# AI4Science-WestlakeU/wdno

Measured on AMD Instinct MI355X. Metric: diffusion train steps/sec, 2D smoke U-Net (8 samples per GPU per step), higher is better.
Workload: dtype f32

## Files before the change

### include/wdno_hip.h

```cpp
#ifndef WDNO_HIP_H
#define WDNO_HIP_H
#include <stdint.h>
#include <stddef.h>

#ifdef __cplusplus
extern "C" {
#endif

typedef void* wdno_stream_t;

enum { WDNO_OK = 0, WDNO_EINVAL = -1, WDNO_ELAUNCH = -2, WDNO_EUNSUPPORTED = -3, WDNO_EWORKSPACE = -4 };

#define WDNO_AMAX_SLOTS 64
#define WDNO_AMAX_STRIDE 16
#define WDNO_AMAX_FLOATS (WDNO_AMAX_SLOTS * WDNO_AMAX_STRIDE)
const char* wdno_strerror(int code);
int wdno_version(void);
const char* wdno_last_hip_error(void);
int wdno_set_debug(int mode);

typedef struct {
  int nd;
  int mode;
  int L;
// ... 81 lines not shown
int wdno_conv_wgrad_f16x3_param(const void* xh, const void* xl, const float* sx, const void* dyh, const void* dyl, const float* sdy,
                                const void* pixel_table, float* dw, int Kn, int Cn, void* ws, size_t ws_bytes,
                                const wdno_conv_geom* g, wdno_stream_t s);
#define WDNO_WGRAD_REDUCE_MAX 40
typedef struct wdno_wgrad_reduce_item {
  const float* ws; float* dw;
  int n, splits;
  int K8, C8, kw, ntap, Kn, Cn;
  int tiled;
  int reserved;
} wdno_wgrad_reduce_item;
int wdno_conv_wgrad_partials(const void* xh, const void* xl, const float* sx, const void* dyh, const void* dyl, const float* sdy,
                             const void* pixel_table, float* dw, int Kn, int Cn, void* ws, size_t ws_bytes,
                             const wdno_conv_geom* g, wdno_wgrad_reduce_item* item, wdno_stream_t s);
int wdno_wgrad_reduce_multi(const wdno_wgrad_reduce_item* items, int n_items, wdno_stream_t s);
size_t wdno_conv_wgrad_ws_bytes(const wdno_conv_geom* g);
int wdno_conv_wgrad(const float* x, const float* dy, float* dwp, void* ws, size_t ws_bytes,
                    const wdno_conv_geom* g, wdno_stream_t s);
#define WDNO_ROWS_SUM_MAX 64
typedef struct wdno_rows_sum_item {
  const void* part; float* out;
  int rows, stride, col0, ncols;
  int is_double, reserved;
} wdno_rows_sum_item;
int wdno_rows_sum_multi(const wdno_rows_sum_item* items, int n_items, wdno_stream_t s);
size_t wdno_colsum_ws_bytes(int64_t P, int C);
int wdno_colsum(const float* in, float* out, int64_t P, int C, void* ws, size_t ws_bytes, wdno_stream_t s);

int wdno_cast_bf16(const float* x, void* out16, int64_t rows, int C, int C8, wdno_stream_t s);
int wdno_cast_bf16_colsum(const float* x, void* out16, float* colsum_out, void* ws, size_t ws_bytes, int64_t rows, int C, int C8, wdno_stream_t s);
// ... 307 lines not shown
```

### wdno_amd/_lib.py

```python
import contextlib
import ctypes as C
import os

import torch

HERE = os.path.dirname(os.path.abspath(__file__))
LIB_PATH = os.path.join(HERE, 'libwdno_hip.so')

P = C.c_void_p
I = C.c_int
L = C.c_int64
F = C.c_float
Z = C.c_size_t


class DwtDesc(C.Structure):
    _fields_ = [('nd', I), ('mode', I), ('L', I), ('n_img', I), ('in_dims', I * 3), ('out_dims', I * 3),
                ('cs_img', L), ('cs_band', L), ('cs0', L), ('cs1', L)]


class ConvGeom(C.Structure):
    _fields_ = [(k, I) for k in ('N', 'D', 'H', 'W', 'C', 'OD', 'OH', 'OW', 'K', 'kd', 'kh', 'kw', 'sd', 'sh', 'sw',
                                 'pd', 'ph', 'pw', 'YD', 'YH', 'YW', 'osd', 'osh', 'osw', 'ood', 'ooh', 'oow')]

# ... 23 lines not shown
ATTN_FAMILIES = ('mfma24', 'mfma', 'mfma64', 'tiled', 'tiled_staged', 'tiled_unstaged', 'big', 'rows')


class LinAttnPlan(C.Structure):
    _fields_ = [(k, I) for k in ('kstats_chunks', 'ctx_chunks', 'token_tiles', 'family', 'rc')]


class LayerNormPlan(C.Structure):
    _fields_ = [(k, I) for k in ('tpr', 'vpl', 'rows_per_block', 'blocks', 'max_rows_walk', 'rc')]


class ConvWgradPlan(C.Structure):
    _fields_ = [(k, I) for k in ('family', 'bm', 'bn', 'splits', 'pix_per_split', 'splitpair', 'reduce_tiled', 'items', 'grid')]


CONV_FAMILIES = ('fp32', 'h3', 'h3d', 'h3t', 'h3t_stem')
WGRAD_FAMILIES = ('h3', 'h3d', 'h3w', 'h3s')


class RowsSumItem(C.Structure):
    _fields_ = [('part', C.c_void_p), ('out', C.c_void_p), ('rows', I), ('stride', I), ('col0', I), ('ncols', I), ('is_double', I), ('reserved', I)]


class BurgersDesc(C.Structure):
    _fields_ = [(k, I) for k in ('N', 's', 'nx0', 'nt_f', 'nxf', 'steps', 'record_time', 'f_time', 'num_t', 'sub_s', 'out_cols', 'waves',
                                 'points')] + [(k, F) for k in ('c', 'd', 'dm', 'dt')]


class BurgersGenerateDesc(C.Structure):
    _fields_ = [(k, I) for k in ('N', 's', 't', 'steps', 'record_time', 'f_time', 'num_t', 'st', 'sx', 'f_rows', 'cols', 'waves', 'points',
# ... 75 lines not shown
    'wdno_amax_multi': (I, [P, I, I, P]),
    'wdno_pack_split_weight_multi': (I, [P, I, I, P]),
    'wdno_conv_fwd_f16x3': (I, [P, P, P, P, P, P, P, P, P, PG, P]),
    'wdno_conv_fwd_f16x3_amax': (I, [P, P, P, P, P, P, P, P, P, P, PG, P]),
    'wdno_conv_fwd_f16x3_ws': (I, [P, P, P, P, P, P, P, P, P, P, PG, P, Z, P]),
    'wdno_conv_fwd_split_ws_bytes': (Z, [PG]),
    'wdno_conv_wgrad_f16x3_ws_bytes': (Z, [PG]),
    'wdno_conv_fwd_plan': (I, [PG, I, I, Z, P]),
    'wdno_conv_wgrad_plan': (I, [PG, I, I, I, P]),
    'wdno_conv_pixel_table': (I, [P, PG, P]),
    'wdno_conv_wgrad_f16x3': (I, [P, P, P, P, P, P, P, P, P, Z, PG, P]),
    'wdno_conv_wgrad_f16x3_param': (I, [P, P, P, P, P, P, P, P, I, I, P, Z, PG, P]),
    'wdno_conv_wgrad_partials': (I, [P, P, P, P, P, P, P, P, I, I, P, Z, PG, P, P]),
    'wdno_wgrad_reduce_multi': (I, [P, I, P]),
    'wdno_rows_sum_multi': (I, [P, I, P]),
    'wdno_cast_bf16': (I, [P, P, L, I, I, P]),
    'wdno_cast_bf16_colsum': (I, [P, P, P, P, Z, L, I, I, P]),
    'wdno_conv_fwd_bf16': (I, [P, P, P, P, P, P, PG, P]),
    'wdno_conv_fwd_f16x3_zbox': (I, [P, P, P, P, P, P, P, P, P, P, PG, P, P]),
    'wdno_conv_fwd_bf16_ex': (I, [P, P, P, P, P, I, P, PG, P, P]),
    'wdno_conv_wgrad_bf16_param': (I, [P, P, P, P, I, I, P, Z, PG, P]),
    'wdno_conv_wgrad_ws_bytes': (Z, [PG]),
    'wdno_conv_wgrad': (I, [P, P, P, P, Z, PG, P]),
    'wdno_colsum_ws_bytes': (Z, [L, I]),
    'wdno_colsum': (I, [P, P, L, I, P, Z, P]),
    'wdno_groupnorm_ws_bytes': (Z, [L, L, I, I]),
    'wdno_groupnorm_stats_floats': (Z, [L, I, I]),
    'wdno_groupnorm_act_fwd': (I, [P, P, P, P, P, P, L, L, I, I, F, I, P, Z, P]),
    'wdno_groupnorm_act_fwd_amax': (I, [P, P, P, P, P, P, P, L, L, I, I, F, I, P, Z, P]),
    'wdno_groupnorm_act_bwd': (I, [P, P, P, P, P, P, P, P, P, L, L, I, I, I, P, Z, P]),
# ... 131 lines not shown
```

### wdno_amd/csrc/conv_common.h

```cpp
#pragma once
#include "common.h"

typedef float f32x16 __attribute__((ext_vector_type(16)));

#define BK 32
#define LDS_STRIDE 36

struct ConvP {
  wdno_conv_geom g;
  int R;
  int nchunk;
  int nsteps;
  int64_t P;
  int identity_out;
  int debug;
  int tiles_n;
  int ntiles;
  int ksplit;
  float* amax_rec;
  int tsplit;
  float* split_ws;
  size_t split_ws_bytes;
  int zb_blocks, zb_d, zb_h;
  int out_bf16;
// ... 17 lines not shown
static inline int check_geom(const wdno_conv_geom* g) {
  if (!g) return WDNO_EINVAL;
  if (g->N <= 0 || g->D <= 0 || g->H <= 0 || g->W <= 0 || g->C <= 0 || g->K <= 0) return WDNO_EINVAL;
  if (g->OD <= 0 || g->OH <= 0 || g->OW <= 0 || g->kd <= 0 || g->kh <= 0 || g->kw <= 0) return WDNO_EINVAL;
  if (g->sd <= 0 || g->sh <= 0 || g->sw <= 0 || g->osd <= 0 || g->osh <= 0 || g->osw <= 0) return WDNO_EINVAL;
  if ((g->C & 3) || (g->K & 3)) return WDNO_EUNSUPPORTED;
  if ((g->OD - 1) * g->osd + g->ood >= g->YD || (g->OH - 1) * g->osh + g->ooh >= g->YH || (g->OW - 1) * g->osw + g->oow >= g->YW)
    return WDNO_EINVAL;
  return WDNO_OK;
}
#include "debug_modes.h"
void wdno_wgrad_h3d_plan(const wdno_conv_geom* g, int* bm, int* bn, int* splits, int* pix_per_split, int* splitpair = nullptr);
int wdno_conv_wgrad_h3_dma(const void* xh, const void* xl, const void* dyh, const void* dyl, const float* sx, const float* sdy,
                           const void* table, float* wsf, const wdno_conv_geom* g, hipStream_t st);
int wdno_wgrad_h3d_describe(const wdno_conv_geom* g, wdno_wgrad_plan* out);
struct ConvFwdChoice {
  wdno_conv_plan plan;
  int kw;
  int sp;
};
static inline int conv_persistent_grid(int64_t items) {
  int grid = wdno_num_cus() & ~7;
  if (grid < 8) grid = 8;
  if (items < grid) grid = (int)items;
  return grid;
}
int wdno_conv_fwd_fp32_plan(const wdno_conv_geom* g, wdno_conv_plan* out);
int wdno_conv_fwd_h3_dma_choose(const ConvP& p, bool lp, ConvFwdChoice& c);
int wdno_conv_fwd_h3_dma(const void* xh, const void* xl, const void* wh, const void* wl, const float* sx, const float* sw,
                         const float* bias, const float* residual, float* y, ConvP& p, const ConvFwdChoice& c, hipStream_t st);
// ... 36 lines not shown
```

### wdno_amd/csrc/conv_h3.hip

```cpp
#include "conv_common.h"
#include <type_traits>
#include <algorithm>

typedef _Float16 half8 __attribute__((ext_vector_type(8)));
typedef __bf16 bf16x8 __attribute__((ext_vector_type(8)));
template <bool LP>
__device__ __forceinline__ f32x16 mfma_16(half8 a, half8 b, f32x16 c) {
  if constexpr (LP) return __builtin_amdgcn_mfma_f32_32x32x16_bf16(__builtin_bit_cast(bf16x8, a), __builtin_bit_cast(bf16x8, b), c, 0, 0, 0);
  else return __builtin_amdgcn_mfma_f32_32x32x16_f16(a, b, c, 0, 0, 0);
}

#define HBK 32
#define HST 40

template <bool RECORD>
__global__ __launch_bounds__(256) void amax_kernel(const float* __restrict__ x, int64_t n, unsigned* __restrict__ out) {
  __shared__ float red[4];
  const int64_t n4 = n >> 2;
  const float4* x4 = reinterpret_cast<const float4*>(x);
  float m = 0.f;
  const int64_t stride = (int64_t)gridDim.x * 1024;
  for (int64_t k0 = (int64_t)blockIdx.x * 1024 + threadIdx.x; k0 < n4; k0 += stride) {
    float4 v[4];
#pragma unroll
// ... 1107 lines not shown
  return wdno_check_launch();
}

extern "C" int wdno_conv_wgrad_partials(const void* xh, const void* xl, const float* sx, const void* dyh, const void* dyl, const float* sdy,
                                        const void* pixel_table, float* dw, int Kn, int Cn, void* ws, size_t ws_bytes,
                                        const wdno_conv_geom* g, wdno_wgrad_reduce_item* item, wdno_stream_t s) {
  WDNO_REQUIRE(g && item && dw && Kn > 0 && Cn > 0 && Kn <= g->K && Cn <= g->C);
  int splits = 0;
  int rc = wgrad_h3_partials(xh, xl, sx, dyh, dyl, sdy, pixel_table, nullptr, ws, ws_bytes, g, as_stream(s), &splits);
  if (rc) return rc;
  const int64_t n = (int64_t)g->kd * g->kh * g->K * (int64_t)g->kw * g->C;
  if (n >= 0x7fffffff) return WDNO_EUNSUPPORTED;
  item->ws = (const float*)ws; item->dw = dw; item->n = (int)n; item->splits = splits; item->K8 = g->K; item->C8 = g->C; item->kw = g->kw;
  item->ntap = g->kd * g->kh; item->Kn = Kn; item->Cn = Cn; item->tiled = wgrad_h3_reduce_tiled(splits, g, Kn, Cn) ? 1 : 0;
  return wdno_check_launch();
}

extern "C" int wdno_conv_wgrad_bf16_param(const void* x16, const void* dy16, const void* pixel_table, float* dw, int Kn, int Cn, void* ws,
                                          size_t ws_bytes, const wdno_conv_geom* g, wdno_stream_t s) {
  WDNO_REQUIRE(g && Kn > 0 && Cn > 0 && Kn <= g->K && Cn <= g->C);
  hipStream_t st = as_stream(s);
  int splits = 0;
  int rc = wgrad_h3_partials(x16, nullptr, nullptr, dy16, nullptr, nullptr, pixel_table, nullptr, ws, ws_bytes, g, st, &splits);
  if (rc) return rc;
  const int64_t n = (int64_t)g->kd * g->kh * g->K * (int64_t)g->kw * g->C;
  wgrad_h3_reduce_launch((const float*)ws, dw, n, splits, g, Kn, Cn, st);
  return wdno_check_launch();
}

#define PS_LDS_FLOATS 10240
// ... 170 lines not shown
```

### wdno_amd/csrc/conv_wgrad_h3d.hip

```cpp
#include "conv_common.h"
#include <type_traits>

typedef _Float16 half8 __attribute__((ext_vector_type(8)));
typedef __bf16 bf16x8 __attribute__((ext_vector_type(8)));
typedef int int4v __attribute__((ext_vector_type(4)));
#define WD_OOB 0x7ffffff0
template <bool LP>
__device__ __forceinline__ f32x16 mfma_16(half8 a, half8 b, f32x16 c) {
  if constexpr (LP) return __builtin_amdgcn_mfma_f32_32x32x16_bf16(__builtin_bit_cast(bf16x8, a), __builtin_bit_cast(bf16x8, b), c, 0, 0, 0);
  else return __builtin_amdgcn_mfma_f32_32x32x16_f16(a, b, c, 0, 0, 0);
}

struct WgradDP {
  ConvP c;
  int tiles_k, tiles_r, splits, nsteps;
  int items;
  int pix_per_split;
  int xcd_chunk;
  int splitpair, n_a;
};

__device__ __forceinline__ int4v wd_rsrc(const void* ptr, unsigned bytes) {
  uint64_t a = reinterpret_cast<uint64_t>(ptr);
  int4v r;
// ... 12 lines not shown
  return v;
}
template <int NCH>
__device__ __forceinline__ half8 wd_frag(const char* plane, int lane_off, int pix0, int ch0) {
  typedef short short4v __attribute__((ext_vector_type(4)));
  typedef short4v __attribute__((address_space(3))) * lds_s4;
  const char* p0 = plane + lane_off + (pix0 / 4) * (NCH * 64) + (ch0 / 32) * 256;
  short4v a = __builtin_amdgcn_ds_read_tr16_b64_v4i16((lds_s4)(p0));
  short4v b = __builtin_amdgcn_ds_read_tr16_b64_v4i16((lds_s4)(p0 + NCH * 64));
  typedef short short8v __attribute__((ext_vector_type(8)));
  short8v c = __builtin_shufflevector(a, b, 0, 1, 2, 3, 4, 5, 6, 7);
  return __builtin_bit_cast(half8, c);
}

template <int BM, int BN, int NS, bool LP>
__global__ __launch_bounds__(512) void conv_wgrad_h3d_kernel(const _Float16* __restrict__ xh, const _Float16* __restrict__ xl,
                                                              const _Float16* __restrict__ dyh, const _Float16* __restrict__ dyl,
                                                              const float* __restrict__ sx, const float* __restrict__ sdy,
                                                              const int4v* __restrict__ table, float* __restrict__ ws, WgradDP wp,
                                                              unsigned x_bytes, unsigned dy_bytes, unsigned tbl_bytes) {
  constexpr int TM = BM / 64, TN = BN / 64;
  constexpr int ACH = BM / 8, BCH = BN / 8;
  constexpr int A_PLANE = 32 * ACH * 16, B_PLANE = 32 * BCH * 16;
  constexpr int NPL = LP ? 1 : 2;
  constexpr int A_LO = A_PLANE, B_HI = NPL * A_PLANE, B_LO = B_HI + B_PLANE;
  constexpr int STAGE = NPL * (A_PLANE + B_PLANE);
  constexpr int APC = A_PLANE / 1024, BPC = B_PLANE / 1024;
  constexpr int NPAIR = APC + BPC;
  static_assert(NPAIR % 4 == 0, "pieces are dealt to four producer waves");
  constexpr int R = NPAIR / 4;
  constexpr int PW = NPL * R;
  constexpr int LA = 2;
  static_assert(R + (NS - 2) * (R + PW) <= 63, "vmcnt is a 6-bit counter");
  extern __shared__ __attribute__((aligned(1024))) char smem[];
  const ConvP& p = wp.c;
  const wdno_conv_geom& g = p.g;
  const int tid = threadIdx.x;
  const int wave = __builtin_amdgcn_readfirstlane(tid >> 6), lane = tid & 63;
  int it_first, it_stride, my_items;
  if (wp.xcd_chunk > 0) {
    const int xcd = (int)blockIdx.x & 7, idx = (int)blockIdx.x >> 3;
    const int beg = xcd * wp.xcd_chunk, end = min(beg + wp.xcd_chunk, wp.items);
    it_stride = (int)gridDim.x >> 3;
    it_first = beg + idx;
    my_items = it_first < end ? (end - it_first + it_stride - 1) / it_stride : 0;
  } else {
    it_first = (int)blockIdx.x; it_stride = (int)gridDim.x;
    my_items = (wp.items - it_first + it_stride - 1) / it_stride;
  }
  const int ntap = g.kd * g.kh;
  auto decode_item = [&](int t, int& tile_k, int& tap, int& tile_r, int& split) {
    int id = it_first + t * it_stride;
    tile_r = id % wp.tiles_r; id /= wp.tiles_r;
    tap = id % ntap; id /= ntap;
    tile_k = id % wp.tiles_k;
    split = id / wp.tiles_k;
  };

  if (wave >= 4) {
    const int pq = wave - 4;
    int4v rxh = wd_rsrc(xh, x_bytes), rxl = wd_rsrc(xl, x_bytes), rdh = wd_rsrc(dyh, dy_bytes), rdl = wd_rsrc(dyl, dy_bytes);
    int4v rtb = wd_rsrc(table, tbl_bytes);
// ... 222 lines not shown
      float* orow = out + (int64_t)kk * p.R;
#pragma unroll
      for (int b = 0; b < TN; ++b) {
#pragma unroll
        for (int e4 = 0; e4 < 4; ++e4) {
          const int rr = tile_r * BN + n_base + b * 32 + 8 * e4 + 4 * hh;
          if (rr < p.R)
            *reinterpret_cast<float4*>(orow + rr) = make_float4(acc[a][b][4 * e4] * inv, acc[a][b][4 * e4 + 1] * inv, acc[a][b][4 * e4 + 2] * inv, acc[a][b][4 * e4 + 3] * inv);
        }
      }
    }
  }
}

template <int NS, bool LP>
__global__ __launch_bounds__(512) void conv_wgrad_h3w_kernel(const _Float16* __restrict__ xh, const _Float16* __restrict__ xl,
                                                              const _Float16* __restrict__ dyh, const _Float16* __restrict__ dyl,
                                                              const float* __restrict__ sx, const float* __restrict__ sdy,
                                                              const int4v* __restrict__ table, float* __restrict__ ws, WgradDP wp,
                                                              unsigned x_bytes, unsigned dy_bytes, unsigned tbl_bytes) {
  constexpr int KW = 3, BM = 64, CT = 64;
  constexpr int TM = 2, TN = 3;
  constexpr int ACH = BM / 8, XCH = CT / 8;
  constexpr int XROWS = 32 + KW - 1;
  constexpr int A_PLANE = 32 * ACH * 16, W_PLANE = 5 * 1024, B_PLANE = 2 * W_PLANE;
  constexpr int ZROWS = 9 * (XCH * 64);
  constexpr int NDY = 2;
  constexpr int NPL = LP ? 1 : 2;
  constexpr int A_LO = NDY * A_PLANE, B_HI = NPL * NDY * A_PLANE, B_LO = B_HI + B_PLANE;
  constexpr int STAGE = NPL * (NDY * A_PLANE + B_PLANE);
  constexpr int APC = A_PLANE / 1024, WPC = W_PLANE / 1024;
  static_assert(APC == 4 && WPC == 5, "ordinary items: pairs 0-3 dy, 4-8 window 0, 9-13 window 1; split-pair items: 0-3 dy 0, 4-7 dy 1, 8-12 window 0, 13-17 window 1");
  constexpr int LA = 2;
  extern __shared__ __attribute__((aligned(1024))) char smem[];
  const ConvP& p = wp.c;
  const wdno_conv_geom& g = p.g;
  const int tid = threadIdx.x;
  const int wave = __builtin_amdgcn_readfirstlane(tid >> 6), lane = tid & 63;
  int it_first, it_stride, my_items;
  if (wp.xcd_chunk > 0) {
    const int xcd = (int)blockIdx.x & 7, idx = (int)blockIdx.x >> 3;
    const int beg = xcd * wp.xcd_chunk, end = min(beg + wp.xcd_chunk, wp.items);
    it_stride = (int)gridDim.x >> 3;
    it_first = beg + idx;
    my_items = it_first < end ? (end - it_first + it_stride - 1) / it_stride : 0;
  } else {
    it_first = (int)blockIdx.x; it_stride = (int)gridDim.x;
    my_items = (wp.items - it_first + it_stride - 1) / it_stride;
  }
  const int ntap = g.kd * g.kh, npair = wp.splitpair ? ntap >> 1 : (ntap + 1) >> 1;
  auto decode_item = [&](int t, int& tile_k, int& tile_c, int (&tp)[2], int (&sp)[2]) {
    int id = it_first + t * it_stride;
    if (id < wp.n_a) {
      tile_c = id % wp.tiles_r; id /= wp.tiles_r;
      const int q = id % npair; id /= npair;
      tile_k = id % wp.tiles_k;
      sp[0] = sp[1] = id / wp.tiles_k;
      tp[0] = 2 * q; tp[1] = 2 * q + 1;
    } else {
      id -= wp.n_a;
      tile_c = id % wp.tiles_r; id /= wp.tiles_r;
      tile_k = id % wp.tiles_k;
// ... 57 lines not shown
            i_off[j] = k * 2;
          } else {
            i_ok[j] = row[j] < XROWS;
            i_off[j] = g.pw * g.C + tc * CT + chk[j];
          }
        }
      };
      if (my_items > 0) { load_item_r(); load_item_p(); }
      int4v rec[LA + 1][R];
      bool rok[LA + 1][R];
      auto fetch = [&](auto SLOT) {
        constexpr int S = decltype(SLOT)::value;
        const bool live = rc.t < my_items;
#pragma unroll
        for (int j = 0; j < R; ++j) {
          const int pm = r_pbeg[slot[j]] + rc.s * 32 + row[j] - (pq + 4 * j < APCT ? 0 : g.pw);
          rok[S][j] = live && pm >= 0 && pm < (int)p.P;
          rec[S][j] = wd_load_rec(rtb, rok[S][j] ? pm * 16 : WD_OOB);
        }
        if (live && ++rc.s == wp.nsteps) { rc.s = 0; if (++rc.t < my_items) load_item_r(); }
      };
      auto issue = [&](auto SLOT, int stage) {
        constexpr int S = decltype(SLOT)::value;
        const bool live = pc.t < my_items;
        const unsigned sb = lds0 + stage * STAGE;
        const int k2 = g.K * 2;
#pragma unroll
        for (int j = 0; j < R; ++j) {
          int4v e = rec[S][j];
          asm volatile("" : "+v"(e));
          const int gp = pq + 4 * j;
// ... 213 lines not shown
              *reinterpret_cast<float4*>(orow + rr) = make_float4(acc[a][b][4 * e4] * inv, acc[a][b][4 * e4 + 1] * inv, acc[a][b][4 * e4 + 2] * inv, acc[a][b][4 * e4 + 3] * inv);
            }
          }
        }
      }
    }
  };
  if (whalf == 0) run(std::integral_constant<int, 0>{});
  else run(std::integral_constant<int, 1>{});
}

#ifndef WDNO_H3S_STAGES
#define WDNO_H3S_STAGES 4
#endif
template <bool LP>
__global__ __launch_bounds__(512) void conv_wgrad_h3s_kernel(const _Float16* __restrict__ xh, const _Float16* __restrict__ xl,
                                                              const _Float16* __restrict__ dyh, const _Float16* __restrict__ dyl,
                                                              const float* __restrict__ sx, const float* __restrict__ sdy,
                                                              float* __restrict__ ws, WgradDP wp, unsigned x_bytes, unsigned dy_bytes) {
  constexpr int KW = 7, CX = 48, NS = WDNO_H3S_STAGES, TM = 2;
  constexpr int ROWB = CX * 2, XROWS = 32 + KW - 1, X_DATA = XROWS * ROWB;
  constexpr int A_PLANE = 4096, X_PLANE = 4096, ZADDR = X_DATA;
  constexpr int NPL = LP ? 1 : 2;
  constexpr int A_LO = A_PLANE, B_HI = NPL * A_PLANE, B_LO = B_HI + X_PLANE;
  constexpr int STAGE = NPL * (A_PLANE + X_PLANE);
  constexpr int PER = 2 * NPL;
  extern __shared__ __attribute__((aligned(1024))) char smem[];
  const ConvP& p = wp.c;
  const wdno_conv_geom& g = p.g;
  const int tid = threadIdx.x;
  const int wave = __builtin_amdgcn_readfirstlane(tid >> 6), lane = tid & 63;
  int it_first, it_stride, my_items;
  if (wp.xcd_chunk > 0) {
    const int xcd = (int)blockIdx.x & 7, idx = (int)blockIdx.x >> 3;
    const int beg = xcd * wp.xcd_chunk, end = min(beg + wp.xcd_chunk, wp.items);
    it_stride = (int)gridDim.x >> 3;
    it_first = beg + idx;
    my_items = it_first < end ? (end - it_first + it_stride - 1) / it_stride : 0;
  } else {
    it_first = (int)blockIdx.x; it_stride = (int)gridDim.x;
    my_items = (wp.items - it_first + it_stride - 1) / it_stride;
  }
  const int ntap = g.kd * g.kh;
  const int total = my_items * wp.nsteps;

  if (wave >= 4) {
    const int pq = wave - 4;
    int4v rxh = wd_rsrc(xh, x_bytes), rxl = wd_rsrc(xl, x_bytes), rdh = wd_rsrc(dyh, dy_bytes), rdl = wd_rsrc(dyl, dy_bytes);
    asm volatile("s_nop 4" : "+s"(rxh), "+s"(rxl), "+s"(rdh), "+s"(rdl));
    const unsigned lds0 = __builtin_amdgcn_readfirstlane((unsigned)(size_t)(__attribute__((address_space(3))) char*)smem);
    const int f = 64 * pq + lane;
    const int xr = f / (ROWB / 16), xc = f - xr * (ROWB / 16);
    const bool x_slot = xr < XROWS;
    const int gi = f >> 5, du = (f >> 4) & 1, dj = (f >> 2) & 3, dc = f & 3;
    const int dpix = 16 * (gi >> 2) + 8 * ((gi >> 1) & 1) + (gi & 1) + 2 * dj;
// ... 172 lines not shown
        for (int b = 0; b < TN; ++b) {
#pragma unroll
          for (int e4 = 0; e4 < 4; ++e4) {
            const int rr = 32 * (tb0 + b) + 8 * e4 + 4 * hh;
            if (rr < p.R)
              *reinterpret_cast<float4*>(orow + rr) = make_float4(acc[a][b][4 * e4] * inv, acc[a][b][4 * e4 + 1] * inv, acc[a][b][4 * e4 + 2] * inv, acc[a][b][4 * e4 + 3] * inv);
          }
        }
      }
    }
  };
  if (wave < 3) run(std::integral_constant<int, 3>{});
  else run(std::integral_constant<int, 2>{});
}

static bool wd_window_takes(const wdno_conv_geom* g) {
  if (wdno_debug_mode == WDNO_DBG_CHUNKED_DMA_CONV || (wdno_debug_mode == WDNO_DBG_PER_AXIS_DWT_AND_WGRAD_WINDOW_K64 && g->K > 64)) return false;
  return g->sd == 1 && g->sh == 1 && g->sw == 1 && g->OD == g->D && g->OH == g->H && g->OW == g->W && g->kw == 3 && g->pw == 1 &&
         (g->C % 64) == 0 && (g->K % 8) == 0;
}
static bool wd_stem_takes(const wdno_conv_geom* g) {
  if (wdno_debug_mode == WDNO_DBG_CHUNKED_DMA_CONV) return false;
  return g->sd == 1 && g->sh == 1 && g->sw == 1 && g->OD == g->D && g->OH == g->H && g->OW == g->W && g->kw == 7 && g->pw == 3 &&
         g->C == 48 && (g->K % 8) == 0 && g->K <= 64 && g->kd <= 8 && g->kh <= 8;
}
void wdno_wgrad_h3d_plan(const wdno_conv_geom* g, int* bm, int* bn, int* splits, int* pix_per_split, int* splitpair) {
  ConvP c;
  fill_params(c, g);
  if (splitpair) *splitpair = 0;
  if (wd_stem_takes(g)) {
// ... 154 lines not shown
    return WDNO_OK;
  }
  if (xl == nullptr) {
    if (bm == 128 && bn == 192) launch_wd<128, 192, true>(xh, xh, dyh, dyh, sx, sdy, table, wsf, w, st);
    else if (bm == 128) launch_wd<128, 128, true>(xh, xh, dyh, dyh, sx, sdy, table, wsf, w, st);
    else if (bn == 192) launch_wd<64, 192, true>(xh, xh, dyh, dyh, sx, sdy, table, wsf, w, st);
    else launch_wd<64, 128, true>(xh, xh, dyh, dyh, sx, sdy, table, wsf, w, st);
    return WDNO_OK;
  }
  if (bm == 128 && bn == 192) launch_wd<128, 192, false>(xh, xl, dyh, dyl, sx, sdy, table, wsf, w, st);
  else if (bm == 128) launch_wd<128, 128, false>(xh, xl, dyh, dyl, sx, sdy, table, wsf, w, st);
  else if (bn == 192) launch_wd<64, 192, false>(xh, xl, dyh, dyl, sx, sdy, table, wsf, w, st);
  else launch_wd<64, 128, false>(xh, xl, dyh, dyl, sx, sdy, table, wsf, w, st);
  return WDNO_OK;
}
```

### wdno_amd/ops.py

```python
import contextlib
import ctypes as C
import math
import os

import torch

from . import _lib
from ._lib import AttnDesc, CondDesc, ConvGeom, DwtDesc

WEIGHT_EPOCH = 0
_pack_cache = {}


PROFILE = None


class _timed:

    def __init__(self, key, flops):
        self.key, self.flops = key, flops

    def __enter__(self):
        if PROFILE is not None:
            self.e0 = torch.cuda.Event(enable_timing=True)
# ... 545 lines not shown
        _wtables[keys] = tabs
    amax, at, stt, nw = tabs
    lib = _lib_()
    with torch.no_grad():
        if not lp:
            amax.zero_()
            _lib.check(lib.wdno_amax_multi(_p(at), nw, 64, _stream()), 'amax_multi')
        _lib.check(lib.wdno_pack_split_weight_multi(_p(stt), len(keys), 256, _stream()), 'pack_split_weight_multi')
    for k in keys:
        pl = _wplans[k]
        pl.ver = (pl.w._version, WEIGHT_EPOCH)


def cache_snapshot():
    return [dict(_pack_cache), dict(_wplans), dict(_wtables), dict(_lin_tables), dict(_rot_cache), dict(_pixel_tables), dict(_freq_cache),
            {k: v[0] for k, v in _amax_pool.items()}]


def captured_plans(since=None):
    return [pl for pl in _wplans.values() if since is None or pl.used >= since]


def touch_plans(plans):
    e = WEIGHT_EPOCH
    for pl in plans:
        pl.used = e


def prepare_graph_refresh():
    epoch = WEIGHT_EPOCH
    for pl in _wplans.values():
        if pl.used >= epoch - 3:
            pl.used = epoch
    bump_weight_epoch(params=False)
    if _wplans:
        for lp in {pl.lp for pl in _wplans.values()}:
            _refresh_weight_plans(WEIGHT_EPOCH, lp)
    bump_weight_epoch(params=False)


def split_weight(w, kind, cp8, kp, pack=None):
    lp = _lp()
    key = (w.data_ptr(), kind, cp8, kp, tuple(w.shape), tuple(w.stride()), lp)
    ver = (w._version, WEIGHT_EPOCH)
# ... 172 lines not shown
        return 'conv_wgrad_h3s_kernel<64,352>'
    if window:
        return 'conv_wgrad_h3w_kernel<64,384>'
    cdiv = lambda a, b: -(-a // b)
    bn = 192 if cdiv(run, 192) * 192 <= cdiv(run, 128) * 128 else 128
    return f'conv_wgrad_h3d_kernel<{128 if k > 64 else 64},{bn}>'


FLAT_WGRAD = True
_FLAT_ARMED = False
DEFER_WGRAD_REDUCE = True
_WGRAD_PENDING = None
WGRAD_FLUSH_BYTES = int(os.environ.get('WDNO_WGRAD_FLUSH_MB', '0')) << 20
DEFER_ROW_SUMS = True
_ROWSUM_PENDING = []
_DEFERRED_DSTS = set()


def flush_wgrad_reduces():
    global _WGRAD_PENDING, _ROWSUM_PENDING
    pend, rows = _WGRAD_PENDING, _ROWSUM_PENDING
    if rows:
        _ROWSUM_PENDING = []
        ritems = (_lib.RowsSumItem * len(rows))(*[it for it, _ in rows])
        _lib.check(_lib_().wdno_rows_sum_multi(C.cast(ritems, C.c_void_p), len(rows), _stream()), 'rows_sum_multi')
        _DEFERRED_DSTS.update(int(it.out) for it, _ in rows)
    if not pend:
        return
    _WGRAD_PENDING = [] if _FLAT_ARMED else None
    items = (_lib.WgradReduceItem * len(pend))(*[it for it, _ in pend])
    _lib.check(_lib_().wdno_wgrad_reduce_multi(C.cast(items, C.c_void_p), len(pend), _stream()), 'wgrad_reduce_multi')
    _DEFERRED_DSTS.update(int(it.dw) for it, _ in pend)


class _RowsJob:
    __slots__ = ('keep', 'ptr', 'rows', 'stride', 'col0', 'ncols', 'is_double')

    def __init__(self, keep, ptr, rows, stride, col0, ncols, is_double):
        self.keep, self.ptr, self.rows, self.stride, self.col0, self.ncols, self.is_double = keep, ptr, rows, stride, col0, ncols, is_double

    def item(self, out, ncols=None):
        it = _lib.RowsSumItem()
        it.part, it.out, it.rows, it.stride, it.col0 = self.ptr, out.data_ptr(), self.rows, self.stride, self.col0
        it.ncols, it.is_double, it.reserved = self.ncols if ncols is None else ncols, self.is_double, 0
        return it


# ... 56 lines not shown
    table = _pixel_tables.get(tkey)
    if table is None:
        table = torch.empty((n * osp[0] * osp[1] * osp[2], 4), device=xh.device, dtype=torch.int32)
        _lib.check(lib.wdno_conv_pixel_table(_p(table), C.byref(g), _stream()), 'conv_pixel_table')
        _pixel_tables[tkey] = table
    flops = 2.0 * n * osp[0] * osp[1] * osp[2] * k8 * ks[0] * ks[1] * ks[2] * c8
    if LAUNCH_LOG is not None:
        LAUNCH_LOG.append(('wgrad', _geom_fields(g), xl is None, param_kc))
    window = tuple(st) == (1, 1, 1) and tuple(osp) == (d, h, ww) and ks[2] == 3 and pd[2] == 1 and c8 % 64 == 0
    if tuple(st) == (1, 1, 1) and tuple(osp) == (d, h, ww) and ks[2] == 7 and pd[2] == 3 and c8 == 48 and k8 <= 64 and max(ks) <= 8:
        window = 'stem'
    if param_kc is not None and out is not None and _WGRAD_PENDING is not None:
        kn, cn = param_kc
        dw = out
        item = _lib.WgradReduceItem()
        with _timed(_wgrad_h3_kernel_name(k8, ks[2] * c8, window), flops):
            _lib.check(lib.wdno_conv_wgrad_partials(_p(xh), _p(xl), _p(sx), _p(gh), _p(gl), _p(sg), _p(table), _p(dw), kn, cn, _p(ws), nb, C.byref(g),
                                                    C.byref(item), _stream()), 'conv_wgrad_partials')
        _WGRAD_PENDING.append((item, ws))
        if WGRAD_FLUSH_BYTES and sum(w.numel() for _, w in _WGRAD_PENDING) > WGRAD_FLUSH_BYTES:
            flush_wgrad_reduces()
        return dw
    if xl is None:
        assert param_kc is not None
        kn, cn = param_kc
        dw = out if out is not None else torch.empty((kn, cn, *ks), device=xh.device, dtype=torch.float32)
        with _timed(_wgrad_h3_kernel_name(k8, ks[2] * c8, window), flops):
            _lib.check(lib.wdno_conv_wgrad_bf16_param(_p(xh), _p(gh), _p(table), _p(dw), kn, cn, _p(ws), nb, C.byref(g), _stream()), 'conv_wgrad_bf16_param')
        return dw
    if param_kc is not None:
# ... 1190 lines not shown
```

Measured before the change: 33.20.

## Batch deferred conv weight-gradient launches into grouped multi-descriptor kernels

Weight-gradient partial kernels are no longer launched one per layer. Each is recorded as a device descriptor and deferred until the reduce flush, then launched as one persistent kernel per family and tile config that loops over the descriptors. The aim is to cut per-kernel launch overhead and the gaps between many small wgrad kernels. In exchange, jobs run serially inside a block with a __syncthreads between them, and the grid is the largest one in the group. It also needs descriptor tables uploaded through a pinned staging buffer during graph capture, and jobs are reordered in reverse.

```diff
diff --git a/include/wdno_hip.h b/include/wdno_hip.h
--- a/include/wdno_hip.h
+++ b/include/wdno_hip.h
@@ -119,6 +119,13 @@
                              const void* pixel_table, float* dw, int Kn, int Cn, void* ws, size_t ws_bytes,
                              const wdno_conv_geom* g, wdno_wgrad_reduce_item* item, wdno_stream_t s);
 int wdno_wgrad_reduce_multi(const wdno_wgrad_reduce_item* items, int n_items, wdno_stream_t s);
+#define WDNO_WGRAD_MULTI_DESC_BYTES 384
+int wdno_conv_wgrad_job(const void* xh, const void* xl, const float* sx, const void* dyh, const void* dyl, const float* sdy,
+                        const void* pixel_table, float* dw, int Kn, int Cn, void* ws, size_t ws_bytes, const wdno_conv_geom* g,
+                        void* desc, wdno_wgrad_reduce_item* item, wdno_wgrad_plan* plan);
+int wdno_conv_wgrad_h3d_multi(const void* descs, int n, int grid, int bm, int bn, int lowp, wdno_stream_t s);
+int wdno_conv_wgrad_h3w_multi(const void* descs, int n, int grid, int lowp, wdno_stream_t s);
+int wdno_conv_wgrad_h3s_multi(const void* descs, int n, int grid, int lowp, wdno_stream_t s);
 size_t wdno_conv_wgrad_ws_bytes(const wdno_conv_geom* g);
 int wdno_conv_wgrad(const float* x, const float* dy, float* dwp, void* ws, size_t ws_bytes,
                     const wdno_conv_geom* g, wdno_stream_t s);
diff --git a/wdno_amd/_lib.py b/wdno_amd/_lib.py
--- a/wdno_amd/_lib.py
+++ b/wdno_amd/_lib.py
@@ -61,6 +61,7 @@
     _fields_ = [(k, I) for k in ('family', 'bm', 'bn', 'splits', 'pix_per_split', 'splitpair', 'reduce_tiled', 'items', 'grid')]
 
 
+WGRAD_MULTI_DESC_BYTES = 384
 CONV_FAMILIES = ('fp32', 'h3', 'h3d', 'h3t', 'h3t_stem')
 WGRAD_FAMILIES = ('h3', 'h3d', 'h3w', 'h3s')
 
@@ -166,6 +167,10 @@
     'wdno_conv_wgrad_partials': (I, [P, P, P, P, P, P, P, P, I, I, P, Z, PG, P, P]),
     'wdno_wgrad_reduce_multi': (I, [P, I, P]),
     'wdno_rows_sum_multi': (I, [P, I, P]),
+    'wdno_conv_wgrad_job': (I, [P, P, P, P, P, P, P, P, I, I, P, Z, PG, P, P, P]),
+    'wdno_conv_wgrad_h3d_multi': (I, [P, I, I, I, I, I, P]),
+    'wdno_conv_wgrad_h3w_multi': (I, [P, I, I, I, P]),
+    'wdno_conv_wgrad_h3s_multi': (I, [P, I, I, I, P]),
     'wdno_cast_bf16': (I, [P, P, L, I, I, P]),
     'wdno_cast_bf16_colsum': (I, [P, P, P, P, Z, L, I, I, P]),
     'wdno_conv_fwd_bf16': (I, [P, P, P, P, P, P, PG, P]),
diff --git a/wdno_amd/csrc/conv_common.h b/wdno_amd/csrc/conv_common.h
--- a/wdno_amd/csrc/conv_common.h
+++ b/wdno_amd/csrc/conv_common.h
@@ -55,6 +55,9 @@
 int wdno_conv_wgrad_h3_dma(const void* xh, const void* xl, const void* dyh, const void* dyl, const float* sx, const float* sdy,
                            const void* table, float* wsf, const wdno_conv_geom* g, hipStream_t st);
 int wdno_wgrad_h3d_describe(const wdno_conv_geom* g, wdno_wgrad_plan* out);
+int wdno_wgrad_h3d_multi_desc(const void* xh, const void* xl, const void* dyh, const void* dyl, const float* sx, const float* sdy,
+                              const void* table, float* wsf, const wdno_conv_geom* g, void* desc, int* family, int* bm, int* bn, int* grid);
+int wdno_wgrad_h3d_multi_launch(int family, int bm, int bn, int lowp, const void* descs, int n, int grid, hipStream_t st);
 struct ConvFwdChoice {
   wdno_conv_plan plan;
   int kw;
diff --git a/wdno_amd/csrc/conv_h3.hip b/wdno_amd/csrc/conv_h3.hip
--- a/wdno_amd/csrc/conv_h3.hip
+++ b/wdno_amd/csrc/conv_h3.hip
@@ -1145,6 +1145,48 @@
   item->ws = (const float*)ws; item->dw = dw; item->n = (int)n; item->splits = splits; item->K8 = g->K; item->C8 = g->C; item->kw = g->kw;
   item->ntap = g->kd * g->kh; item->Kn = Kn; item->Cn = Cn; item->tiled = wgrad_h3_reduce_tiled(splits, g, Kn, Cn) ? 1 : 0;
   return wdno_check_launch();
+}
+
+extern "C" int wdno_conv_wgrad_job(const void* xh, const void* xl, const float* sx, const void* dyh, const void* dyl, const float* sdy,
+                                   const void* pixel_table, float* dw, int Kn, int Cn, void* ws, size_t ws_bytes, const wdno_conv_geom* g,
+                                   void* desc, wdno_wgrad_reduce_item* item, wdno_wgrad_plan* plan) {
+  WDNO_REQUIRE(g && item && plan && desc && dw && xh && dyh && ws && Kn > 0 && Cn > 0 && Kn <= g->K && Cn <= g->C);
+  WDNO_REQUIRE((xl == nullptr) == (dyl == nullptr));
+  int rc = check_geom(g);
+  if (rc) return rc;
+  if ((g->C & 7) || (g->K & 7) || !pixel_table || wdno_debug_mode != 0) return WDNO_EUNSUPPORTED;
+  if ((int64_t)g->N * g->D * g->H * g->W * g->C * 2 >= OOB_OFFSET || (int64_t)g->N * g->YD * g->YH * g->YW * g->K * 2 >= OOB_OFFSET)
+    return WDNO_EUNSUPPORTED;
+  WgradHP w;
+  rc = wgrad_h3_choose(g, w, *plan);
+  if (rc) return rc;
+  if (plan->family == WDNO_WGRAD_REG_H3) return WDNO_EUNSUPPORTED;
+  const int64_t n = (int64_t)g->kd * g->kh * g->K * (int64_t)g->kw * g->C;
+  if (n >= 0x7fffffff) return WDNO_EUNSUPPORTED;
+  if (ws_bytes < (size_t)plan->splits * (size_t)n * sizeof(float)) return WDNO_EWORKSPACE;
+  int family, bm, bn, grid;
+  rc = wdno_wgrad_h3d_multi_desc(xh, xl, dyh, dyl, sx, sdy, pixel_table, (float*)ws, g, desc, &family, &bm, &bn, &grid);
+  if (rc) return rc;
+  if (family != plan->family || bm != plan->bm || bn != plan->bn || grid != plan->grid) return WDNO_EINVAL;
+  plan->reduce_tiled = wgrad_h3_reduce_tiled(plan->splits, g, Kn, Cn) ? 1 : 0;
+  item->ws = (const float*)ws; item->dw = dw; item->n = (int)n; item->splits = plan->splits; item->K8 = g->K; item->C8 = g->C; item->kw = g->kw;
+  item->ntap = g->kd * g->kh; item->Kn = Kn; item->Cn = Cn; item->tiled = plan->reduce_tiled; item->reserved = 0;
+  return WDNO_OK;
+}
+extern "C" int wdno_conv_wgrad_h3d_multi(const void* descs, int n, int grid, int bm, int bn, int lowp, wdno_stream_t s) {
+  WDNO_REQUIRE(descs);
+  int rc = wdno_wgrad_h3d_multi_launch(WDNO_WGRAD_CHUNKED_H3D, bm, bn, lowp, descs, n, grid, as_stream(s));
+  return rc ? rc : wdno_check_launch();
+}
+extern "C" int wdno_conv_wgrad_h3w_multi(const void* descs, int n, int grid, int lowp, wdno_stream_t s) {
+  WDNO_REQUIRE(descs);
+  int rc = wdno_wgrad_h3d_multi_launch(WDNO_WGRAD_WINDOW_H3W, 64, 192, lowp, descs, n, grid, as_stream(s));
+  return rc ? rc : wdno_check_launch();
+}
+extern "C" int wdno_conv_wgrad_h3s_multi(const void* descs, int n, int grid, int lowp, wdno_stream_t s) {
+  WDNO_REQUIRE(descs);
+  int rc = wdno_wgrad_h3d_multi_launch(WDNO_WGRAD_STEM_H3S, 64, 352, lowp, descs, n, grid, as_stream(s));
+  return rc ? rc : wdno_check_launch();
 }
 
 extern "C" int wdno_conv_wgrad_bf16_param(const void* x16, const void* dy16, const void* pixel_table, float* dw, int Kn, int Cn, void* ws,
diff --git a/wdno_amd/csrc/conv_wgrad_h3d.hip b/wdno_amd/csrc/conv_wgrad_h3d.hip
--- a/wdno_amd/csrc/conv_wgrad_h3d.hip
+++ b/wdno_amd/csrc/conv_wgrad_h3d.hip
@@ -1,4 +1,5 @@
 #include "conv_common.h"
+#include <string.h>
 #include <type_traits>
 
 typedef _Float16 half8 __attribute__((ext_vector_type(8)));
@@ -50,11 +51,11 @@
 }
 
 template <int BM, int BN, int NS, bool LP>
-__global__ __launch_bounds__(512) void conv_wgrad_h3d_kernel(const _Float16* __restrict__ xh, const _Float16* __restrict__ xl,
-                                                              const _Float16* __restrict__ dyh, const _Float16* __restrict__ dyl,
-                                                              const float* __restrict__ sx, const float* __restrict__ sdy,
-                                                              const int4v* __restrict__ table, float* __restrict__ ws, WgradDP wp,
-                                                              unsigned x_bytes, unsigned dy_bytes, unsigned tbl_bytes) {
+__device__ __forceinline__ void conv_wgrad_h3d_body(const _Float16* __restrict__ xh, const _Float16* __restrict__ xl,
+                                                    const _Float16* __restrict__ dyh, const _Float16* __restrict__ dyl,
+                                                    const float* __restrict__ sx, const float* __restrict__ sdy,
+                                                    const int4v* __restrict__ table, float* __restrict__ ws, const WgradDP wp,
+                                                    unsigned x_bytes, unsigned dy_bytes, unsigned tbl_bytes, int bid, int nblk) {
   constexpr int TM = BM / 64, TN = BN / 64;
   constexpr int ACH = BM / 8, BCH = BN / 8;
   constexpr int A_PLANE = 32 * ACH * 16, B_PLANE = 32 * BCH * 16;
@@ -75,13 +76,13 @@
   const int wave = __builtin_amdgcn_readfirstlane(tid >> 6), lane = tid & 63;
   int it_first, it_stride, my_items;
   if (wp.xcd_chunk > 0) {
-    const int xcd = (int)blockIdx.x & 7, idx = (int)blockIdx.x >> 3;
+    const int xcd = bid & 7, idx = bid >> 3;
     const int beg = xcd * wp.xcd_chunk, end = min(beg + wp.xcd_chunk, wp.items);
-    it_stride = (int)gridDim.x >> 3;
+    it_stride = nblk >> 3;
     it_first = beg + idx;
     my_items = it_first < end ? (end - it_first + it_stride - 1) / it_stride : 0;
   } else {
-    it_first = (int)blockIdx.x; it_stride = (int)gridDim.x;
+    it_first = bid; it_stride = nblk;
     my_items = (wp.items - it_first + it_stride - 1) / it_stride;
   }
   const int ntap = g.kd * g.kh;
@@ -334,11 +335,11 @@
 }
 
 template <int NS, bool LP>
-__global__ __launch_bounds__(512) void conv_wgrad_h3w_kernel(const _Float16* __restrict__ xh, const _Float16* __restrict__ xl,
-                                                              const _Float16* __restrict__ dyh, const _Float16* __restrict__ dyl,
-                                                              const float* __restrict__ sx, const float* __restrict__ sdy,
-                                                              const int4v* __restrict__ table, float* __restrict__ ws, WgradDP wp,
-                                                              unsigned x_bytes, unsigned dy_bytes, unsigned tbl_bytes) {
+__device__ __forceinline__ void conv_wgrad_h3w_body(const _Float16* __restrict__ xh, const _Float16* __restrict__ xl,
+                                                    const _Float16* __restrict__ dyh, const _Float16* __restrict__ dyl,
+                                                    const float* __restrict__ sx, const float* __restrict__ sdy,
+                                                    const int4v* __restrict__ table, float* __restrict__ ws, const WgradDP wp,
+                                                    unsigned x_bytes, unsigned dy_bytes, unsigned tbl_bytes, int bid, int nblk) {
   constexpr int KW = 3, BM = 64, CT = 64;
   constexpr int TM = 2, TN = 3;
   constexpr int ACH = BM / 8, XCH = CT / 8;
@@ -359,13 +360,13 @@
   const int wave = __builtin_amdgcn_readfirstlane(tid >> 6), lane = tid & 63;
   int it_first, it_stride, my_items;
   if (wp.xcd_chunk > 0) {
-    const int xcd = (int)blockIdx.x & 7, idx = (int)blockIdx.x >> 3;
+    const int xcd = bid & 7, idx = bid >> 3;
     const int beg = xcd * wp.xcd_chunk, end = min(beg + wp.xcd_chunk, wp.items);
-    it_stride = (int)gridDim.x >> 3;
+    it_stride = nblk >> 3;
     it_first = beg + idx;
     my_items = it_first < end ? (end - it_first + it_stride - 1) / it_stride : 0;
   } else {
-    it_first = (int)blockIdx.x; it_stride = (int)gridDim.x;
+    it_first = bid; it_stride = nblk;
     my_items = (wp.items - it_first + it_stride - 1) / it_stride;
   }
   const int ntap = g.kd * g.kh, npair = wp.splitpair ? ntap >> 1 : (ntap + 1) >> 1;
@@ -453,7 +454,7 @@
         const bool live = rc.t < my_items;
 #pragma unroll
         for (int j = 0; j < R; ++j) {
-          const int pm = r_pbeg[slot[j]] + rc.s * 32 + row[j] - (pq + 4 * j < APCT ? 0 : g.pw);
+          const int pm = (slot[j] ? r_pbeg[1] : r_pbeg[0]) + rc.s * 32 + row[j] - (pq + 4 * j < APCT ? 0 : g.pw);
           rok[S][j] = live && pm >= 0 && pm < (int)p.P;
           rec[S][j] = wd_load_rec(rtb, rok[S][j] ? pm * 16 : WD_OOB);
         }
@@ -697,10 +698,10 @@
 #define WDNO_H3S_STAGES 4
 #endif
 template <bool LP>
-__global__ __launch_bounds__(512) void conv_wgrad_h3s_kernel(const _Float16* __restrict__ xh, const _Float16* __restrict__ xl,
-                                                              const _Float16* __restrict__ dyh, const _Float16* __restrict__ dyl,
-                                                              const float* __restrict__ sx, const float* __restrict__ sdy,
-                                                              float* __restrict__ ws, WgradDP wp, unsigned x_bytes, unsigned dy_bytes) {
+__device__ __forceinline__ void conv_wgrad_h3s_body(const _Float16* __restrict__ xh, const _Float16* __restrict__ xl,
+                                                    const _Float16* __restrict__ dyh, const _Float16* __restrict__ dyl,
+                                                    const float* __restrict__ sx, const float* __restrict__ sdy,
+                                                    float* __restrict__ ws, const WgradDP wp, unsigned x_bytes, unsigned dy_bytes, int bid, int nblk) {
   constexpr int KW = 7, CX = 48, NS = WDNO_H3S_STAGES, TM = 2;
   constexpr int ROWB = CX * 2, XROWS = 32 + KW - 1, X_DATA = XROWS * ROWB;
   constexpr int A_PLANE = 4096, X_PLANE = 4096, ZADDR = X_DATA;
@@ -715,13 +716,13 @@
   const int wave = __builtin_amdgcn_readfirstlane(tid >> 6), lane = tid & 63;
   int it_first, it_stride, my_items;
   if (wp.xcd_chunk > 0) {
-    const int xcd = (int)blockIdx.x & 7, idx = (int)blockIdx.x >> 3;
+    const int xcd = bid & 7, idx = bid >> 3;
     const int beg = xcd * wp.xcd_chunk, end = min(beg + wp.xcd_chunk, wp.items);
-    it_stride = (int)gridDim.x >> 3;
+    it_stride = nblk >> 3;
     it_first = beg + idx;
     my_items = it_first < end ? (end - it_first + it_stride - 1) / it_stride : 0;
   } else {
-    it_first = (int)blockIdx.x; it_stride = (int)gridDim.x;
+    it_first = bid; it_stride = nblk;
     my_items = (wp.items - it_first + it_stride - 1) / it_stride;
   }
   const int ntap = g.kd * g.kh;
@@ -924,6 +925,71 @@
   else run(std::integral_constant<int, 2>{});
 }
 
+template <int BM, int BN, int NS, bool LP>
+__global__ __launch_bounds__(512) void conv_wgrad_h3d_kernel(const _Float16* __restrict__ xh, const _Float16* __restrict__ xl,
+                                                              const _Float16* __restrict__ dyh, const _Float16* __restrict__ dyl,
+                                                              const float* __restrict__ sx, const float* __restrict__ sdy,
+                                                              const int4v* __restrict__ table, float* __restrict__ ws, WgradDP wp,
+                                                              unsigned x_bytes, unsigned dy_bytes, unsigned tbl_bytes) {
+  conv_wgrad_h3d_body<BM, BN, NS, LP>(xh, xl, dyh, dyl, sx, sdy, table, ws, wp, x_bytes, dy_bytes, tbl_bytes, (int)blockIdx.x, (int)gridDim.x);
+}
+template <int NS, bool LP>
+__global__ __launch_bounds__(512) void conv_wgrad_h3w_kernel(const _Float16* __restrict__ xh, const _Float16* __restrict__ xl,
+                                                              const _Float16* __restrict__ dyh, const _Float16* __restrict__ dyl,
+                                                              const float* __restrict__ sx, const float* __restrict__ sdy,
+                                                              const int4v* __restrict__ table, float* __restrict__ ws, WgradDP wp,
+                                                              unsigned x_bytes, unsigned dy_bytes, unsigned tbl_bytes) {
+  conv_wgrad_h3w_body<NS, LP>(xh, xl, dyh, dyl, sx, sdy, table, ws, wp, x_bytes, dy_bytes, tbl_bytes, (int)blockIdx.x, (int)gridDim.x);
+}
+template <bool LP>
+__global__ __launch_bounds__(512) void conv_wgrad_h3s_kernel(const _Float16* __restrict__ xh, const _Float16* __restrict__ xl,
+                                                              const _Float16* __restrict__ dyh, const _Float16* __restrict__ dyl,
+                                                              const float* __restrict__ sx, const float* __restrict__ sdy,
+                                                              float* __restrict__ ws, WgradDP wp, unsigned x_bytes, unsigned dy_bytes) {
+  conv_wgrad_h3s_body<LP>(xh, xl, dyh, dyl, sx, sdy, ws, wp, x_bytes, dy_bytes, (int)blockIdx.x, (int)gridDim.x);
+}
+
+struct WgradMultiDesc {
+  const _Float16 *xh, *xl, *dyh, *dyl;
+  const float *sx, *sdy;
+  const int4v* table;
+  float* ws;
+  WgradDP wp;
+  unsigned x_bytes, dy_bytes, tbl_bytes;
+  int grid;
+};
+static_assert(sizeof(WgradMultiDesc) <= WDNO_WGRAD_MULTI_DESC_BYTES && WDNO_WGRAD_MULTI_DESC_BYTES % 16 == 0, "descriptor slot (include/wdno_hip.h)");
+__device__ __forceinline__ const WgradMultiDesc* wd_desc(const char* descs, int i) {
+  return reinterpret_cast<const WgradMultiDesc*>(descs + (size_t)i * WDNO_WGRAD_MULTI_DESC_BYTES);
+}
+template <int BM, int BN, int NS, bool LP>
+__global__ __launch_bounds__(512) void conv_wgrad_h3d_multi_kernel(const char* __restrict__ descs, int n) {
+  for (int i = 0; i < n; ++i) {
+    const WgradMultiDesc d = *wd_desc(descs, i);
+    if ((int)blockIdx.x < d.grid)
+      conv_wgrad_h3d_body<BM, BN, NS, LP>(d.xh, d.xl, d.dyh, d.dyl, d.sx, d.sdy, d.table, d.ws, d.wp, d.x_bytes, d.dy_bytes, d.tbl_bytes, (int)blockIdx.x, d.grid);
+    __syncthreads();
+  }
+}
+template <int NS, bool LP>
+__global__ __launch_bounds__(512) void conv_wgrad_h3w_multi_kernel(const char* __restrict__ descs, int n) {
+  for (int i = 0; i < n; ++i) {
+    const WgradMultiDesc d = *wd_desc(descs, i);
+    if ((int)blockIdx.x < d.grid)
+      conv_wgrad_h3w_body<NS, LP>(d.xh, d.xl, d.dyh, d.dyl, d.sx, d.sdy, d.table, d.ws, d.wp, d.x_bytes, d.dy_bytes, d.tbl_bytes, (int)blockIdx.x, d.grid);
+    __syncthreads();
+  }
+}
+template <bool LP>
+__global__ __launch_bounds__(512) void conv_wgrad_h3s_multi_kernel(const char* __restrict__ descs, int n) {
+  for (int i = 0; i < n; ++i) {
+    const WgradMultiDesc d = *wd_desc(descs, i);
+    if ((int)blockIdx.x < d.grid)
+      conv_wgrad_h3s_body<LP>(d.xh, d.xl, d.dyh, d.dyl, d.sx, d.sdy, d.ws, d.wp, d.x_bytes, d.dy_bytes, (int)blockIdx.x, d.grid);
+    __syncthreads();
+  }
+}
+
 static bool wd_window_takes(const wdno_conv_geom* g) {
   if (wdno_debug_mode == WDNO_DBG_CHUNKED_DMA_CONV || (wdno_debug_mode == WDNO_DBG_PER_AXIS_DWT_AND_WGRAD_WINDOW_K64 && g->K > 64)) return false;
   return g->sd == 1 && g->sh == 1 && g->sw == 1 && g->OD == g->D && g->OH == g->H && g->OW == g->W && g->kw == 3 && g->pw == 1 &&
@@ -1108,3 +1174,64 @@
   else launch_wd<64, 128, false>(xh, xl, dyh, dyl, sx, sdy, table, wsf, w, st);
   return WDNO_OK;
 }
+
+int wdno_wgrad_h3d_multi_desc(const void* xh, const void* xl, const void* dyh, const void* dyl, const float* sx, const float* sdy,
+                              const void* table, float* wsf, const wdno_conv_geom* g, void* desc, int* family, int* bm, int* bn, int* grid) {
+  WgradMultiDesc d;
+  memset(&d, 0, sizeof(d));
+  int rc = wd_choose(g, d.wp, *bm, *bn, *family);
+  if (rc) return rc;
+  const bool lp = xl == nullptr;
+  d.xh = (const _Float16*)xh; d.xl = (const _Float16*)(lp ? xh : xl);
+  d.dyh = (const _Float16*)dyh; d.dyl = (const _Float16*)(lp ? dyh : dyl);
+  d.sx = sx; d.sdy = sdy;
+  d.table = (const int4v*)table; d.ws = wsf;
+  d.x_bytes = (unsigned)((int64_t)g->N * g->D * g->H * g->W * g->C * 2);
+  d.dy_bytes = (unsigned)((int64_t)g->N * g->YD * g->YH * g->YW * g->K * 2);
+  d.tbl_bytes = (unsigned)(d.wp.c.P * 16);
+  d.grid = wd_grid(d.wp.items, &d.wp.xcd_chunk);
+  *grid = d.grid;
+  memset(desc, 0, WDNO_WGRAD_MULTI_DESC_BYTES);
+  memcpy(desc, &d, sizeof(d));
+  return WDNO_OK;
+}
+template <typename KERNEL>
+static void wd_multi_launch(KERNEL kernel, bool& attr_done, size_t lds, const void* descs, int n, int grid, hipStream_t st) {
+  if (!attr_done && lds > 64 * 1024) { (void)hipFuncSetAttribute((const void*)kernel, hipFuncAttributeMaxDynamicSharedMemorySize, (int)lds); attr_done = true; }
+  kernel<<<grid, 512, lds, st>>>((const char*)descs, n);
+}
+template <int BM, int BN, bool LP>
+static void launch_wd_multi(const void* descs, int n, int grid, hipStream_t st) {
+  constexpr int NS = 3;
+  static bool done = false;
+  wd_multi_launch(conv_wgrad_h3d_multi_kernel<BM, BN, NS, LP>, done, (size_t)NS * (LP ? 1 : 2) * (32 * (BM / 8) * 16 + 32 * (BN / 8) * 16), descs, n, grid, st);
+}
+int wdno_wgrad_h3d_multi_launch(int family, int bm, int bn, int lowp, const void* descs, int n, int grid, hipStream_t st) {
+  if (n <= 0 || grid <= 0 || grid > wdno_num_cus()) return WDNO_EINVAL;
+  constexpr int NS = 3;
+  if (family == WDNO_WGRAD_STEM_H3S) {
+    static bool done_lp = false, done_sp = false;
+    if (lowp) wd_multi_launch(conv_wgrad_h3s_multi_kernel<true>, done_lp, (size_t)WDNO_H3S_STAGES * (4096 + 4096), descs, n, grid, st);
+    else wd_multi_launch(conv_wgrad_h3s_multi_kernel<false>, done_sp, (size_t)WDNO_H3S_STAGES * 2 * (4096 + 4096), descs, n, grid, st);
+    return WDNO_OK;
+  }
+  if (family == WDNO_WGRAD_WINDOW_H3W) {
+    static bool done_lp = false, done_sp = false;
+    if (lowp) wd_multi_launch(conv_wgrad_h3w_multi_kernel<NS, true>, done_lp, (size_t)NS * (2 * 4096 + 2 * 5120), descs, n, grid, st);
+    else wd_multi_launch(conv_wgrad_h3w_multi_kernel<NS, false>, done_sp, (size_t)NS * 2 * (2 * 4096 + 2 * 5120), descs, n, grid, st);
+    return WDNO_OK;
+  }
+  if (family != WDNO_WGRAD_CHUNKED_H3D || (bm != 64 && bm != 128) || (bn != 128 && bn != 192)) return WDNO_EINVAL;
+  if (lowp) {
+    if (bm == 128 && bn == 192) launch_wd_multi<128, 192, true>(descs, n, grid, st);
+    else if (bm == 128) launch_wd_multi<128, 128, true>(descs, n, grid, st);
+    else if (bn == 192) launch_wd_multi<64, 192, true>(descs, n, grid, st);
+    else launch_wd_multi<64, 128, true>(descs, n, grid, st);
+    return WDNO_OK;
+  }
+  if (bm == 128 && bn == 192) launch_wd_multi<128, 192, false>(descs, n, grid, st);
+  else if (bm == 128) launch_wd_multi<128, 128, false>(descs, n, grid, st);
+  else if (bn == 192) launch_wd_multi<64, 192, false>(descs, n, grid, st);
+  else launch_wd_multi<64, 128, false>(descs, n, grid, st);
+  return WDNO_OK;
+}
diff --git a/wdno_amd/ops.py b/wdno_amd/ops.py
--- a/wdno_amd/ops.py
+++ b/wdno_amd/ops.py
@@ -583,7 +583,7 @@
 
 def cache_snapshot():
     return [dict(_pack_cache), dict(_wplans), dict(_wtables), dict(_lin_tables), dict(_rot_cache), dict(_pixel_tables), dict(_freq_cache),
-            {k: v[0] for k, v in _amax_pool.items()}]
+            {k: v[0] for k, v in _amax_pool.items()}, dict(_wgrad_desc_tables), list(_wgrad_stagings)]
 
 
 def captured_plans(since=None):
@@ -597,6 +597,9 @@
 
 
 def prepare_graph_refresh():
+    global _WGRAD_STAGING
+    if DEFER_WGRAD_LAUNCH:
+        _WGRAD_STAGING = [torch.empty((2 * max(_wgrad_jobs_seen, 64) * _lib.WGRAD_MULTI_DESC_BYTES,), dtype=torch.uint8).pin_memory(), 0]
     epoch = WEIGHT_EPOCH
     for pl in _wplans.values():
         if pl.used >= epoch - 3:
@@ -799,11 +802,19 @@
 WGRAD_FLUSH_BYTES = int(os.environ.get('WDNO_WGRAD_FLUSH_MB', '0')) << 20
 DEFER_ROW_SUMS = True
 _ROWSUM_PENDING = []
+DEFER_WGRAD_LAUNCH = True
+DEFER_WGRAD_STEM = False
+_WGRAD_JOBS = []
+_wgrad_desc_tables = {}
+_wgrad_jobs_seen = 0
+_WGRAD_STAGING = None
+_wgrad_stagings = []
 _DEFERRED_DSTS = set()
 
 
 def flush_wgrad_reduces():
     global _WGRAD_PENDING, _ROWSUM_PENDING
+    _launch_wgrad_jobs()
     pend, rows = _WGRAD_PENDING, _ROWSUM_PENDING
     if rows:
         _ROWSUM_PENDING = []
@@ -816,6 +827,61 @@
     items = (_lib.WgradReduceItem * len(pend))(*[it for it, _ in pend])
     _lib.check(_lib_().wdno_wgrad_reduce_multi(C.cast(items, C.c_void_p), len(pend), _stream()), 'wgrad_reduce_multi')
     _DEFERRED_DSTS.update(int(it.dw) for it, _ in pend)
+
+
+def _wgrad_job_room():
+    if _CAPTURE is None and not torch.cuda.is_current_stream_capturing():
+        return True
+    st = _WGRAD_STAGING
+    return st is not None and st[1] + (len(_WGRAD_JOBS) + 1) * _lib.WGRAD_MULTI_DESC_BYTES <= st[0].numel()
+
+
+def _wgrad_desc_table(key, blob, device):
+    k = (key, blob)
+    tab = _wgrad_desc_tables.get(k)
+    if tab is not None:
+        return tab
+    while len(_wgrad_desc_tables) >= 16:
+        _wgrad_desc_tables.pop(next(iter(_wgrad_desc_tables)))
+    if _CAPTURE is not None or torch.cuda.is_current_stream_capturing():
+        st = _WGRAD_STAGING
+        host = st[0][st[1]:st[1] + len(blob)]
+        st[1] += len(blob)
+        host.copy_(torch.frombuffer(bytearray(blob), dtype=torch.uint8))
+        tab = torch.empty((len(blob),), dtype=torch.uint8, device=device)
+        tab.copy_(host, non_blocking=True)
+        if not any(t is st[0] for t in _wgrad_stagings):
+            _wgrad_stagings.append(st[0])
+            del _wgrad_stagings[:-8]
+    else:
+        tab = torch.frombuffer(bytearray(blob), dtype=torch.uint8).to(device)
+    _wgrad_desc_tables[k] = tab
+    return tab
+
+
+def _launch_wgrad_jobs():
+    global _WGRAD_JOBS, _wgrad_jobs_seen
+    jobs = _WGRAD_JOBS
+    if not jobs:
+        return
+    _WGRAD_JOBS = []
+    _wgrad_jobs_seen = max(_wgrad_jobs_seen, len(jobs))
+    jobs = jobs[::-1]
+    groups = {}
+    for j in jobs:
+        groups.setdefault(j[0], []).append(j)
+    lib = _lib_()
+    dev = jobs[0][3][0].device
+    for key, js in groups.items():
+        family, bm, bn, lp = key
+        tab = _wgrad_desc_table(key, b''.join(j[1] for j in js), dev)
+        grid = max(j[2] for j in js)
+        if family == 1:
+            _lib.check(lib.wdno_conv_wgrad_h3d_multi(_p(tab), len(js), grid, bm, bn, int(lp), _stream()), 'conv_wgrad_h3d_multi')
+        elif family == 2:
+            _lib.check(lib.wdno_conv_wgrad_h3w_multi(_p(tab), len(js), grid, int(lp), _stream()), 'conv_wgrad_h3w_multi')
+        else:
+            _lib.check(lib.wdno_conv_wgrad_h3s_multi(_p(tab), len(js), grid, int(lp), _stream()), 'conv_wgrad_h3s_multi')
 
 
 class _RowsJob:
@@ -902,6 +968,17 @@
         kn, cn = param_kc
         dw = out
         item = _lib.WgradReduceItem()
+        if DEFER_WGRAD_LAUNCH and PROFILE is None and _wgrad_job_room() and (window != 'stem' or DEFER_WGRAD_STEM):
+            desc, plan = C.create_string_buffer(_lib.WGRAD_MULTI_DESC_BYTES), _lib.ConvWgradPlan()
+            rc = lib.wdno_conv_wgrad_job(_p(xh), _p(xl), _p(sx), _p(gh), _p(gl), _p(sg), _p(table), _p(dw), kn, cn, _p(ws), nb, C.byref(g), desc,
+                                         C.byref(item), C.byref(plan))
+            if rc != -3:
+                _lib.check(rc, 'conv_wgrad_job')
+                _WGRAD_JOBS.append(((plan.family, plan.bm, plan.bn, xl is None), desc.raw, plan.grid, (xh, xl, sx, gh, gl, sg, table)))
+                _WGRAD_PENDING.append((item, ws))
+                if WGRAD_FLUSH_BYTES and sum(w.numel() for _, w in _WGRAD_PENDING) > WGRAD_FLUSH_BYTES:
+                    flush_wgrad_reduces()
+                return dw
         with _timed(_wgrad_h3_kernel_name(k8, ks[2] * c8, window), flops):
             _lib.check(lib.wdno_conv_wgrad_partials(_p(xh), _p(xl), _p(sx), _p(gh), _p(gl), _p(sg), _p(table), _p(dw), kn, cn, _p(ws), nb, C.byref(g),
                                                     C.byref(item), _stream()), 'conv_wgrad_partials')
```

Result: no change. 33.31, median of 6 (+0.3%).
